# WHU-USI3DV/LaneMapping

Hardware: AMD Instinct MI355X
Metric: BEV tiles/sec end-to-end (LAS points -> polylines) (higher is better)
Workload: dtype f32; 1 GPU; on-GPU LAS->BEV raster (4,194,304 points/tile resident in HBM) + configs/Proj_polyline_fpn_vit_vertex_2.py, batch=16 per GPU, seeded random weights; lines_per_tile=45, streams=2, hip_graphs=True, points=resident, stream_check=not run (--full runs it), gather_check=n/a (1 rank), raster_check=not run (--full runs it), dist_ranks=1, rccl_ranks=1

## Files before the change

lanemapping_amd/csrc/conv_mfma.hip:

```cpp
#include "common.h"

#include <cstdlib>

typedef float f32x16 __attribute__((ext_vector_type(16)));
typedef float f32x4 __attribute__((ext_vector_type(4)));

namespace {

constexpr int BK = 32;
constexpr int LDS_LD = BK;

__device__ __attribute__((aligned(16))) float g_zero_chunk[4] = {0.f, 0.f, 0.f, 0.f};

struct ConvParams {
    const float* x; const float* wp; const float* scale; const float* shift; const float* res; float* y;
    int ldx, ldr, ldy, res_rows;
    int B, H, W, Cin, Cout, CoutP, Ho, Wo;
    int KH, KW, stride, pad_h, pad_w, dil, act;
    long M;
    const float* zero;
    int taps_real;
    const int* nbr;
    double* gn_part;
    int gn_chunks;
// ... 246 lines not shown
                }
            }
        }
        if (p.gn_part) {
#pragma unroll
            for (int o = LPR; o < 64; o <<= 1)
#pragma unroll
                for (int e = 0; e < 4; ++e) {
                    gs[e] += __shfl_xor(gs[e], o);
                    gq[e] += __shfl_xor(gq[e], o);
                }
            if (lane < LPR) {
                const long hw = (long)p.Ho * p.Wo;
                const long mt = m0 + wm0;
                const long b = mt / hw;
                const long chunk = (mt - b * hw) / WM;
                double* o = p.gn_part + ((b * p.gn_chunks + chunk) * p.Cout + n) * 2;
                for (int e = 0; e < 4 && n + e < p.Cout; ++e) {
                    o[2 * e] = (double)gs[e];
                    o[2 * e + 1] = (double)gq[e];
                }
            }
        }
    }
}

template <int BM, int BN, int WM, int WN, bool GATHER = false, int TPS = 1>
int launch(const ConvParams& p, hipStream_t stream) {
    const size_t kloop = (size_t)2 * (BM + BN) * LDS_LD, stage = (size_t)((BM / WM) * (BN / WN)) * WM * (WN + 4);
    const size_t lds = (kloop > stage ? kloop : stage) * sizeof(float);
    if (int e = lm_ensure_dynamic_lds((const void*)conv_mfma_kernel<BM, BN, WM, WN, GATHER, TPS>, lds)) return e;
    const long m_tiles = (p.M + BM - 1) / BM;
    const long blocks = m_tiles * ((p.Cout + BN - 1) / BN);
    LM_REQUIRE(blocks > 0 && blocks < (1L << 31), "conv_mfma: bad grid %ld", blocks);
    hipLaunchKernelGGL((conv_mfma_kernel<BM, BN, WM, WN, GATHER, TPS>), dim3((unsigned)blocks), dim3((BM / WM) * (BN / WN) * 64), lds, stream, p);
    LM_LAUNCH_CHECK();
    return LM_OK;
}

constexpr int LAT_SLD = 36;
template <int KS, bool RESUP, bool ROWTILE>
__global__ __launch_bounds__(512) void lateral_mfma_kernel(ConvParams p) {
    constexpr int K = KS * 8, SLABS = K / 32, XBUF = 32 * K;
    constexpr int NX = XBUF / 4 / 512;
    static_assert(NX >= 1 && XBUF % (4 * 512) == 0, "whole load passes");
    extern __shared__ __attribute__((aligned(16))) float smem[];
    typedef __attribute__((address_space(1))) const void gptr_t;
    typedef __attribute__((address_space(3))) void lptr_t;
    const int tid = threadIdx.x, lane = tid & 63;
    const int wave = __builtin_amdgcn_readfirstlane(tid >> 6);
    const int j = lane & 31, half = lane >> 5;
    float* const patch = smem + 2 * XBUF + wave * (32 * LAT_SLD);
    f32x4 wf[KS];
    {
        const float* wrow = p.wp + (long)(wave * 32 + j) * p.Cin + 4 * half;
#pragma unroll
        for (int k = 0; k < KS; ++k) wf[k] = *reinterpret_cast<const f32x4*>(wrow + 8 * k);
    }
    const int erow = lane >> 3, n = wave * 32 + (lane & 7) * 4;
    const f32x4 sh = p.shift ? *reinterpret_cast<const f32x4*>(p.shift + n) : f32x4{0.f, 0.f, 0.f, 0.f};
    unsigned yoff[4], roff[4];
#pragma unroll
    for (int q = 0; q < 4; ++q) {
        yoff[q] = (unsigned)((erow + 8 * q) * p.ldy + n) * 4u;
        roff[q] = (unsigned)((erow + 8 * q) * p.ldr + n) * 4u;
    }
    const int ntiles = (int)(p.M >> 5);
    const int xcd = blockIdx.x & 7, wi = blockIdx.x >> 3, nwg = gridDim.x >> 3;
    const int per = (ntiles + 7) >> 3, t_end = min(ntiles, (xcd + 1) * per);
    int tile = xcd * per + wi;
    if (tile >= t_end) return;
    int xoff[NX];
#pragma unroll
    for (int i = 0; i < NX; ++i) {
        const int c = i * 512 + tid, slab = c >> 8, row = (c & 255) >> 3, slot = c & 7;
        xoff[i] = row * p.ldx + slab * 32 + ((slot ^ ((row >> 1) & 7)) << 2);
    }
    auto load_x = [&](int t, int buf) {
        const float* xt = p.x + (long)t * 32 * p.ldx;
#pragma unroll
        for (int i = 0; i < NX; ++i)
            __builtin_amdgcn_global_load_lds((gptr_t*)(xt + xoff[i]), (lptr_t*)(smem + buf * XBUF + (i * 8 + wave) * 256), 16, 0, 0);
    };
    load_x(tile, 0);
    __builtin_amdgcn_s_waitcnt(0x0F70);
    const int fswz = (j >> 1) & 7;
#pragma unroll
    for (int k = 0; k < KS; ++k) asm volatile("" : "+v"(wf[k]));
    for (int it = 0; tile < t_end; tile += nwg, ++it) {
        const int buf = it & 1;
        asm volatile("s_waitcnt vmcnt(4)" ::: "memory");
        __builtin_amdgcn_s_barrier();
        asm volatile("" ::: "memory");
        load_x(min(tile + nwg, t_end - 1), buf ^ 1);
        f32x4 r00[4], r01[4], r10[4], r11[4];
        float wy0[4], wy1[4], wx0[4], wx1[4];
        if (RESUP && ROWTILE) {
            const unsigned mt = (unsigned)__builtin_amdgcn_readfirstlane(tile) * 32u;
            const unsigned t = lm_fastdiv(mt, p.div_wo);
            const int ox0 = (int)(mt - t * p.div_wo.d);
            const int bi = (int)lm_fastdiv(t, p.div_ho);
            const int oy = (int)(t - (unsigned)bi * p.div_ho.d);
            int y0v, y1v;
            float wyav, wybv;
            lm_bilin_axis_scaled(oy, p.res_hi, p.res_sy, y0v, y1v, wyav, wybv);
            const int y0 = __builtin_amdgcn_readfirstlane(y0v), y1 = __builtin_amdgcn_readfirstlane(y1v);
            const float wya = __builtin_bit_cast(float, __builtin_amdgcn_readfirstlane(__builtin_bit_cast(int, wyav)));
            const float wyb = __builtin_bit_cast(float, __builtin_amdgcn_readfirstlane(__builtin_bit_cast(int, wybv)));
            const char* row0 = reinterpret_cast<const char*>(p.res + ((long)bi * p.res_hi + y0) * p.res_wi * p.ldr);
            const char* row1 = reinterpret_cast<const char*>(p.res + ((long)bi * p.res_hi + y1) * p.res_wi * p.ldr);
#pragma unroll
            for (int q = 0; q < 4; ++q) {
                int x0, x1;
                lm_bilin_axis_scaled(ox0 + erow + 8 * q, p.res_wi, p.res_sx, x0, x1, wx0[q], wx1[q]);
                wy0[q] = wya;
                wy1[q] = wyb;
                const unsigned o0 = (unsigned)(x0 * p.ldr + n) * 4u, o1 = (unsigned)(x1 * p.ldr + n) * 4u;
                r00[q] = *reinterpret_cast<const f32x4*>(row0 + o0);
                r01[q] = *reinterpret_cast<const f32x4*>(row0 + o1);
                r10[q] = *reinterpret_cast<const f32x4*>(row1 + o0);
                r11[q] = *reinterpret_cast<const f32x4*>(row1 + o1);
            }
        } else if (RESUP) {
#pragma unroll
            for (int q = 0; q < 4; ++q) {
                const unsigned m = (unsigned)(tile * 32 + erow + 8 * q);
                const unsigned t = lm_fastdiv(m, p.div_wo);
                const int ox = (int)(m - t * p.div_wo.d);
                const int bi = (int)lm_fastdiv(t, p.div_ho);
                const int oy = (int)(t - (unsigned)bi * p.div_ho.d);
                int y0, y1, x0, x1;
                lm_bilin_axis_scaled(oy, p.res_hi, p.res_sy, y0, y1, wy0[q], wy1[q]);
                lm_bilin_axis_scaled(ox, p.res_wi, p.res_sx, x0, x1, wx0[q], wx1[q]);
                const float* rb = p.res + (long)bi * p.res_hi * p.res_wi * p.ldr + n;
                r00[q] = *reinterpret_cast<const f32x4*>(rb + ((long)y0 * p.res_wi + x0) * p.ldr);
                r01[q] = *reinterpret_cast<const f32x4*>(rb + ((long)y0 * p.res_wi + x1) * p.ldr);
                r10[q] = *reinterpret_cast<const f32x4*>(rb + ((long)y1 * p.res_wi + x0) * p.ldr);
                r11[q] = *reinterpret_cast<const f32x4*>(rb + ((long)y1 * p.res_wi + x1) * p.ldr);
            }
        } else if (p.res_rows) {
#pragma unroll
            for (int q = 0; q < 4; ++q) {
                const unsigned m = (unsigned)(tile * 32 + erow + 8 * q);
                r00[q] = *reinterpret_cast<const f32x4*>(p.res + (long)(m - lm_fastdiv(m, p.div_rr) * p.div_rr.d) * p.ldr + n);
            }
        } else {
            const char* rt = reinterpret_cast<const char*>(p.res + (long)__builtin_amdgcn_readfirstlane(tile) * 32 * p.ldr);
#pragma unroll
            for (int q = 0; q < 4; ++q) r00[q] = *reinterpret_cast<const f32x4*>(rt + roff[q]);
        }
        __builtin_amdgcn_sched_barrier(0);
        f32x16 acc;
#pragma unroll
        for (int r = 0; r < 16; ++r) acc[r] = 0.f;
        const float* xb = smem + buf * XBUF + j * 32;
        f32x4 xf = *reinterpret_cast<const f32x4*>(xb + ((half ^ fswz) << 2));
#pragma unroll
        for (int k = 0; k < KS; ++k) {
            f32x4 xn = xf;
            acc = __builtin_amdgcn_mfma_f32_32x32x2f32(wf[k][0], xf[0], acc, 0, 0, 0);
            if (k + 1 < KS) {
                const int fo = (((((k + 1) & 3) << 1) + half) ^ fswz) << 2;
                __builtin_amdgcn_sched_barrier(0);
                xn = *reinterpret_cast<const f32x4*>(xb + ((k + 1) >> 2) * 1024 + fo);
                __builtin_amdgcn_sched_barrier(0);
            }
#pragma unroll
            for (int t = 1; t < 4; ++t) acc = __builtin_amdgcn_mfma_f32_32x32x2f32(wf[k][t], xf[t], acc, 0, 0, 0);
            xf = xn;
        }
        __builtin_amdgcn_sched_barrier(0);
#pragma unroll
        for (int g = 0; g < 4; ++g)
            *reinterpret_cast<f32x4*>(patch + j * LAT_SLD + 8 * g + 4 * half) = f32x4{acc[4 * g], acc[4 * g + 1], acc[4 * g + 2], acc[4 * g + 3]};
        char* const yt = reinterpret_cast<char*>(p.y + (long)__builtin_amdgcn_readfirstlane(tile) * 32 * p.ldy);
#pragma unroll
        for (int q = 0; q < 4; ++q) {
            f32x4 v = *reinterpret_cast<const f32x4*>(patch + (erow + 8 * q) * LAT_SLD + (lane & 7) * 4);
#pragma unroll
            for (int e = 0; e < 4; ++e) v[e] = v[e] + sh[e];
            if (RESUP) {
#pragma unroll
                for (int e = 0; e < 4; ++e) v[e] += lm_bilerp(r00[q][e], r01[q][e], r10[q][e], r11[q][e], wy0[q], wy1[q], wx0[q], wx1[q]);
            } else {
#pragma unroll
                for (int e = 0; e < 4; ++e) v[e] += r00[q][e];
            }
            *reinterpret_cast<f32x4*>(yt + yoff[q]) = v;
        }
    }
}

int lateral_try(const ConvParams& p, hipStream_t stream) {
    static const int on = [] { const char* e = getenv("LM_CONV_LATERAL"); return e ? atoi(e) : 1; }();
    if (!on || p.KH != 1 || p.KW != 1 || p.stride != 1 || p.pad_h != 0 || p.pad_w != 0 || p.Cout != 256 || p.CoutP != 256) return 0;
    if ((p.Cin != 64 && p.Cin != 128) || p.scale || p.act != LM_ACT_NONE || p.gn_part || !p.res) return 0;
    if ((p.ldx & 3) || (p.ldy & 3) || (p.ldr & 3) || p.ldr < p.Cout || p.M >= (1L << 31) - 64 || (p.M & 31)) return 0;
    if (p.res_hi > 0 && p.Cin != 64) return 0;
    if (p.res_hi == 0 && p.Cin != 128) return 0;
    static int cus = 0;
    if (!cus) {
        int dev = 0;
        hipDeviceProp_t prop;
        if (hipGetDevice(&dev) != hipSuccess || hipGetDeviceProperties(&prop, dev) != hipSuccess) return -LM_ERR_HIP;
        cus = prop.multiProcessorCount > 0 ? prop.multiProcessorCount : 256;
    }
    const int ntiles = (int)((p.M + 31) / 32);
    int grid = (cus + 7) / 8 * 8;
    if (grid > (ntiles + 7) / 8 * 8) grid = (ntiles + 7) / 8 * 8;
    const size_t lds = (size_t)(2 * 32 * p.Cin + 8 * 32 * LAT_SLD) * sizeof(float);
#define LM_LAT_LAUNCH(KS, UP, ROW)                                                                                      \
    {                                                                                                                   \
        if (lm_ensure_dynamic_lds((const void*)lateral_mfma_kernel<KS, UP, ROW>, lds)) return -LM_ERR_HIP;              \
        hipLaunchKernelGGL((lateral_mfma_kernel<KS, UP, ROW>), dim3(grid), dim3(512), lds, stream, p);                  \
    }
    if (p.res_hi > 0 && p.Wo % 32 == 0) LM_LAT_LAUNCH(8, true, true)
    else if (p.res_hi > 0) LM_LAT_LAUNCH(8, true, false)
    else LM_LAT_LAUNCH(16, false, false)
#undef LM_LAT_LAUNCH
    if (hipGetLastError() != hipSuccess) return -LM_ERR_HIP;
    return 1;
}

int zero_block(const float** out) {
    static const float* ptr = nullptr;
    if (!ptr) {
        void* sym = nullptr;
        LM_HIP(hipGetSymbolAddress(&sym, HIP_SYMBOL(g_zero_chunk)));
        ptr = (const float*)sym;
    }
    *out = ptr;
    return LM_OK;
}

}

static int conv_dispatch(void* stream, const float* x, int ldx, const float* wp, int CoutP, const float* scale, const float* shift,
                         const float* res, int ldr, int res_rows, float* y, int ldy, int B, int H, int W, int Cin, int Cout,
                         int KH, int KW, int stride, int pad_h, int pad_w, int dil, int act, double* gn_part, int res_hi = 0,
                         int res_wi = 0) {
    LM_REQUIRE(x && wp && y, "conv_mfma: null pointer");
    LM_REQUIRE(Cin > 0 && Cin % BK == 0, "conv_mfma: Cin=%d must be a multiple of %d", Cin, BK);
    LM_REQUIRE(CoutP >= Cout && CoutP % 128 == 0, "conv_mfma: CoutP=%d must be Cout=%d rounded up to 128", CoutP, Cout);
    LM_REQUIRE(ldx >= Cin && ldx % 4 == 0 && ldy >= Cout, "conv_mfma: bad leading dims ldx=%d ldy=%d", ldx, ldy);
    LM_REQUIRE(stride >= 1 && dil >= 1 && KH >= 1 && KW >= 1, "conv_mfma: bad geometry");
    ConvParams p;
    p.x = x; p.wp = wp; p.scale = scale; p.shift = shift; p.res = res; p.y = y;
    p.ldx = ldx; p.ldr = ldr; p.ldy = ldy; p.res_rows = res_rows;
    p.res_hi = res_hi; p.res_wi = res_wi;
    p.B = B; p.H = H; p.W = W; p.Cin = Cin; p.Cout = Cout; p.CoutP = CoutP;
    p.Ho = (H + 2 * pad_h - dil * (KH - 1) - 1) / stride + 1;
    p.Wo = (W + 2 * pad_w - dil * (KW - 1) - 1) / stride + 1;
    LM_REQUIRE(p.Ho > 0 && p.Wo > 0, "conv_mfma: empty output");
    p.KH = KH; p.KW = KW; p.stride = stride; p.pad_h = pad_h; p.pad_w = pad_w; p.dil = dil; p.act = act;
    p.M = (long)B * p.Ho * p.Wo;
    LM_REQUIRE(((long)B * H * W + (long)(KH * dil + pad_h + 1) * W) * ldx < (1L << 31) && (long)KH * KW * CoutP * Cin < (1L << 31),
               "conv_mfma: tensor too large for 32-bit element offsets (B*H*W*ld = %ld)", (long)B * H * W * ldx);
    p.gn_part = gn_part;
    p.gn_chunks = 0;
    p.nbr = nullptr;
    p.taps_real = 0;
    LM_REQUIRE(p.M < (1L << 31) && res_rows >= 0, "conv_mfma: %ld output pixels do not fit 32-bit indices", p.M);
    p.div_wo = lm_fastdiv_make((unsigned)p.Wo);
    p.div_ho = lm_fastdiv_make((unsigned)p.Ho);
    p.div_rr = lm_fastdiv_make((unsigned)(res_rows > 0 ? res_rows : 1));
    p.res_sy = (res_hi > 0 && p.Ho > 1) ? (float)(res_hi - 1) / (float)(p.Ho - 1) : 0.f;
    p.res_sx = (res_wi > 0 && p.Wo > 1) ? (float)(res_wi - 1) / (float)(p.Wo - 1) : 0.f;
    if (int e = zero_block(&p.zero)) return e;
    hipStream_t s = (hipStream_t)stream;
    {
        const int r = lateral_try(p, s);
        if (r < 0) {
            lm_set_error("conv_mfma: lateral kernel launch failed");
            return -r;
        }
        if (r > 0) return LM_OK;
    }
    if (gn_part) {
        LM_REQUIRE(Cout > 64 && Cout % 4 == 0 && ((long)p.Ho * p.Wo) % 128 == 0 && res == nullptr && act == LM_ACT_NONE,
                   "conv_mfma(gn stats): needs Cout > 64, Ho*Wo %% 128 == 0, no residual / activation");
        p.gn_chunks = (int)((long)p.Ho * p.Wo / 64);
        return launch<128, 128, 64, 64>(p, s);
    }
    if (Cout <= 64) return launch<128, 64, 32, 64>(p, s);
    {
        static const long tiny_k = [] { const char* e = getenv("LM_CONV_TINYK"); return e ? atol(e) : 256L; }();
        if ((long)KH * KW * Cin <= tiny_k) return launch<128, 128, 32, 64>(p, s);
    }
    const long big_blocks = ((p.M + 127) / 128) * ((Cout + 127) / 128);
    static const long small_m = [] { const char* e = getenv("LM_CONV_SMALLM"); return e ? atol(e) : 700L; }();
    if (big_blocks < small_m) return launch<64, 64, 32, 32>(p, s);
    return launch<128, 128, 64, 64>(p, s);
}

LM_API int lm_conv2d_nhwc_mfma_f32(void* stream, const float* x, int ldx, const float* wp, int CoutP,
                                   const float* scale, const float* shift,
                                   const float* res, int ldr, int res_rows, float* y, int ldy,
                                   int B, int H, int W, int Cin, int Cout, int KH, int KW,
                                   int stride, int pad_h, int pad_w, int dil, int act) {
    return conv_dispatch(stream, x, ldx, wp, CoutP, scale, shift, res, ldr, res_rows, y, ldy, B, H, W, Cin, Cout, KH, KW, stride,
                         pad_h, pad_w, dil, act, nullptr);
}

LM_API int lm_conv2d_nhwc_mfma_f32_gnstats(void* stream, const float* x, int ldx, const float* wp, int CoutP, const float* shift,
                                           float* y, int ldy, double* gn_partial, int B, int H, int W, int Cin, int Cout,
                                           int KH, int KW, int stride, int pad_h, int pad_w, int dil) {
    LM_REQUIRE(gn_partial, "conv_mfma(gn stats): null partial buffer");
    return conv_dispatch(stream, x, ldx, wp, CoutP, nullptr, shift, nullptr, 0, 0, y, ldy, B, H, W, Cin, Cout, KH, KW, stride,
                         pad_h, pad_w, dil, LM_ACT_NONE, gn_partial);
}

LM_API int lm_conv2d_nhwc_mfma_resup_f32(void* stream, const float* x, int ldx, const float* wp, int CoutP, const float* scale,
                                         const float* shift, const float* res_coarse, int ldr, int Hr, int Wr, float* y, int ldy,
                                         int B, int H, int W, int Cin, int Cout, int KH, int KW, int stride, int pad_h, int pad_w,
                                         int dil, int act) {
    LM_REQUIRE(res_coarse && Hr > 0 && Wr > 0, "conv_mfma(resup): missing coarse residual");
    LM_REQUIRE(Cout % 4 == 0 && ldy % 4 == 0 && ldr % 4 == 0 && ldr >= Cout, "conv_mfma(resup): Cout=%d, ldy=%d, ldr=%d must be multiples of 4", Cout, ldy, ldr);
    const long Ho = (H + 2 * pad_h - dil * (KH - 1) - 1) / stride + 1, Wo = (W + 2 * pad_w - dil * (KW - 1) - 1) / stride + 1;
    LM_REQUIRE((long)B * Ho * Wo < (1L << 31), "conv_mfma(resup): too many output pixels for 32-bit indices");
    return conv_dispatch(stream, x, ldx, wp, CoutP, scale, shift, res_coarse, ldr, 0, y, ldy, B, H, W, Cin, Cout, KH, KW, stride,
                         pad_h, pad_w, dil, act, nullptr, Hr, Wr);
}

LM_API int lm_conv_gather_mfma_f32(void* stream, const float* x, int ldx, const int* nbr, int taps, const float* wp, int CoutP,
                                   const float* scale, const float* shift, const float* res, int ldr, float* y, int ldy,
                                   long M, int Cin, int Cout, int act) {
    LM_REQUIRE(x && nbr && wp && y, "conv_gather: null pointer");
    LM_REQUIRE(M > 0 && taps >= 1, "conv_gather: empty problem (M=%ld taps=%d)", M, taps);
    LM_REQUIRE(Cin == 16 || (Cin > 0 && Cin % BK == 0), "conv_gather: Cin=%d must be 16 or a multiple of %d (zero-pad the feature rows)",
               Cin, BK);
    LM_REQUIRE(CoutP >= Cout && CoutP % 128 == 0, "conv_gather: CoutP=%d must be Cout=%d rounded up to 128", CoutP, Cout);
    LM_REQUIRE(ldx >= Cin && ldx % 4 == 0 && ldy >= Cout, "conv_gather: bad leading dims ldx=%d ldy=%d", ldx, ldy);
    const bool pairs = Cin == 16;
    const int slabs = pairs ? (taps + 1) / 2 : taps;
    ConvParams p;
    p.x = x; p.wp = wp; p.scale = scale; p.shift = shift; p.res = res; p.y = y;
    p.ldx = ldx; p.ldr = ldr; p.ldy = ldy; p.res_rows = 0;
    p.res_hi = 0; p.res_wi = 0;
    p.B = 1; p.H = 1; p.W = 1; p.Cin = pairs ? BK : Cin; p.Cout = Cout; p.CoutP = CoutP; p.Ho = 1; p.Wo = 1;
    p.KH = 1; p.KW = slabs; p.stride = 1; p.pad_h = 0; p.pad_w = 0; p.dil = 1; p.act = act;
    p.M = M;
    LM_REQUIRE(M < (1L << 31) && (long)slabs * CoutP * p.Cin < (1L << 31), "conv_gather: problem too large (M=%ld)", M);
    p.gn_part = nullptr;
    p.gn_chunks = 0;
    p.div_wo = p.div_ho = p.div_rr = lm_fastdiv_make(1);
    p.res_sy = p.res_sx = 0.f;
    p.nbr = nbr;
    p.taps_real = taps;
    if (int e = zero_block(&p.zero)) return e;
    hipStream_t s = (hipStream_t)stream;
    if (pairs) {
        if (Cout <= 32) return launch<128, 32, 32, 32, true, 2>(p, s);
        return launch<128, 64, 32, 64, true, 2>(p, s);
    }
    if (Cout <= 32) return launch<128, 32, 32, 32, true>(p, s);
    if (Cout <= 64) return launch<128, 64, 32, 64, true>(p, s);
    return launch<128, 128, 64, 64, true>(p, s);
}
```

lanemapping_amd/csrc/conv_wino44.hip:

```cpp
#include "common.h"

#include <cstdlib>

typedef float f32x16 __attribute__((ext_vector_type(16)));
typedef float f32x4 __attribute__((ext_vector_type(4)));
typedef float f32x2 __attribute__((ext_vector_type(2)));
typedef _Float16 f16x4 __attribute__((ext_vector_type(4)));
typedef unsigned u32x2 __attribute__((ext_vector_type(2)));

namespace {

__device__ __forceinline__ u32x2 w44_split2(f32x2 t) {
#pragma clang fp contract(off)
    typedef __fp16 f16x2r __attribute__((ext_vector_type(2)));
    const f16x2r h = __builtin_amdgcn_cvt_pkrtz(t[0], t[1]);
    const float h0 = (float)h[0], h1 = (float)h[1];
    const f16x2r l = __builtin_amdgcn_cvt_pkrtz(t[0] - h0, t[1] - h1);
    return u32x2{__builtin_bit_cast(unsigned, h), __builtin_bit_cast(unsigned, l)};
}

constexpr int QBM = 32, QBN = 64, QSEG = 4;
constexpr int QNCELL = 144;
constexpr int QLPW = 14;
constexpr int QGRP = 256 + 8;
constexpr int QRAWF = QLPW * 4 * QGRP;
constexpr int QVF = 36 * 256;
constexpr int QBD = 5, QRING = 6;
static_assert(6 * (QNCELL / 16) * QGRP <= QRAWF && QNCELL % 16 == 0, "patch loads cover the unit");

constexpr unsigned QPADOFF = 0x80000000u;
typedef __amdgpu_buffer_rsrc_t w44_rsrc_t;

struct W44Geom {
    int B, H, W, dil, Ty, Tx;
    int Timg, Tpad;
    long T;
    LmFastDiv dTx, dTy, ddil, dTpad;
};

W44Geom geom44(int B, int H, int W, int dil) {
    W44Geom g;
    g.B = B; g.H = H; g.W = W; g.dil = dil;
    g.Ty = ((H + dil - 1) / dil + 3) / 4;
    g.Tx = ((W + dil - 1) / dil + 3) / 4;
    g.Timg = dil * dil * g.Ty * g.Tx;
    g.Tpad = (g.Timg + QBM - 1) / QBM * QBM;
    g.T = (long)B * g.Tpad;
    g.dTx = lm_fastdiv_make((unsigned)g.Tx); g.dTy = lm_fastdiv_make((unsigned)g.Ty);
    g.ddil = lm_fastdiv_make((unsigned)dil); g.dTpad = lm_fastdiv_make((unsigned)g.Tpad);
    return g;
}

__device__ __forceinline__ void tile44_decode(const W44Geom& g, int t, int& pa, int& pb, int& ty, int& tx) {
    tx = t % g.Tx;
    t /= g.Tx;
    ty = t % g.Ty;
    const int ph = t / g.Ty;
    pa = ph / g.dil;
    pb = ph - pa * g.dil;
}

__device__ __forceinline__ void w44_bt(const float (&d)[6], float (&t)[6]) {
#pragma clang fp contract(off)
    t[0] = __builtin_fmaf(4.f, d[0], __builtin_fmaf(-5.f, d[2], d[4]));
    t[5] = __builtin_fmaf(4.f, d[1], __builtin_fmaf(-5.f, d[3], d[5]));
    const float p = __builtin_fmaf(-4.f, d[2], d[4]), q = __builtin_fmaf(-4.f, d[1], d[3]);
    t[1] = p + q;
    t[2] = p - q;
    const float r = d[4] - d[2], s = d[3] - d[1];
    t[3] = __builtin_fmaf(2.f, s, r);
    t[4] = __builtin_fmaf(-2.f, s, r);
}

__device__ __forceinline__ float w44_fma(float k, float a, float c) { return __builtin_fmaf(k, a, c); }
__device__ __forceinline__ f32x4 w44_fma(float k, f32x4 a, f32x4 c) { return __builtin_elementwise_fma(f32x4{k, k, k, k}, a, c); }
template <typename T>
__device__ __forceinline__ void w44_at(const T (&m)[6], T (&y)[4]) {
#pragma clang fp contract(off)
    const T s1 = m[1] + m[2], d1 = m[1] - m[2], s3 = m[3] + m[4], d3 = m[3] - m[4];
    y[0] = (m[0] + s1) + s3;
    y[1] = w44_fma(2.f, d3, d1);
    y[2] = w44_fma(4.f, s3, s1);
    y[3] = w44_fma(8.f, d3, d1) + m[5];
}

// ... 307 lines not shown
    return 2 * QBD + c;
}
static_assert(q_dma0(17) + q_ndma(17) == QLPW, "the second phase issues every patch load of a unit");

template <bool SPLIT>
__device__ __forceinline__ f32x4 q_aread(const float* v, const float* v1) {
    if constexpr (SPLIT) {
        return f32x4{v[0], v[32], v[128], v[160]};
    } else {
        const f32x2 lo = *reinterpret_cast<const f32x2*>(v), hi = *reinterpret_cast<const f32x2*>(v1);
        return f32x4{lo[0], lo[1], hi[0], hi[1]};
    }
}

__device__ __forceinline__ float* w44_lds_hide(float* p) {
    typedef __attribute__((address_space(3))) float lds_float;
    unsigned a = (unsigned)(unsigned long)(lds_float*)p;
    asm volatile("" : "+v"(a));
    return (float*)(lds_float*)(unsigned long)a;
}

constexpr bool w44_deferred(int S) { return S == 4 || S == 8 || S == 13; }
template <int S>
__device__ __forceinline__ void w44_step_rest(f32x16& acc0, f32x16& acc1, const f32x4 (&b)[2], const f32x4& a_cur) {
    constexpr bool VACC = S % 9 == 8;
    q_mfma<VACC>(acc1, a_cur[0], b[1][0]);
#pragma unroll
    for (int t = 1; t < 4; ++t) {
        q_mfma<VACC>(acc0, a_cur[t], b[0][t]);
        q_mfma<VACC>(acc1, a_cur[t], b[1][t]);
    }
}

template <int S, bool SPLIT>
__device__ __forceinline__ void w44_step(f32x16& acc0, f32x16& acc1, f32x4 (&bq)[QRING][2], unsigned bvoff, const float* bpre,
                                         const float* anext, const float* anext1, const f32x4& a_cur, f32x4& a_nxt, const w44_rsrc_t grsrc, const unsigned (&gvoff)[QLPW], int gsoff,
                                         float* rawld, int wave, W44Xf& xf, const float* const (&col)[6], float* vA, float* vB,
                                         float* vC, bool lower, const W44K& kk) {
    typedef __attribute__((address_space(3))) void lptr_t;
    constexpr int K = S % 9;
    q_bload2(bq[(S + QBD) % QRING], bvoff, bpre);
#pragma unroll
    for (int i = 0; i < q_ndma(S); ++i) {
        constexpr int L0 = q_dma0(S);
        __builtin_amdgcn_raw_ptr_buffer_load_lds(grsrc, (lptr_t*)(rawld + ((L0 + i) * 4 + wave) * QGRP), 16, gvoff[L0 + i], gsoff, 0, 0);
    }
    f32x4 (&b)[2] = bq[S % QRING];
    q_bwait<q_nwait(S)>(b);
    constexpr bool VACC = K == 8;
    const f32x2 a_hi = {a_cur[0], a_cur[1]}, a_lo = {a_cur[2], a_cur[3]};
    if constexpr (SPLIT) q_mfma16<VACC>(acc0, a_hi, f32x2{b[0][0], b[0][1]});
    else q_mfma<VACC>(acc0, a_cur[0], b[0][0]);
    if constexpr (!SPLIT) __builtin_amdgcn_sched_barrier(0);
    if constexpr (K != 4 && K != 8) a_nxt = q_aread<SPLIT>(anext, anext1);
    w44_xf_lds<K, SPLIT>(xf, col, vA, vB, vC);
    if constexpr (!SPLIT) __builtin_amdgcn_sched_barrier(0);
    w44_xf_valu<K>(xf, lower, kk);
    if constexpr (!SPLIT) __builtin_amdgcn_sched_barrier(0);
    if constexpr (SPLIT) {
        q_mfma16<VACC>(acc1, a_hi, f32x2{b[1][0], b[1][1]});
        q_mfma16<VACC>(acc0, a_hi, f32x2{b[0][2], b[0][3]});
        q_mfma16<VACC>(acc1, a_hi, f32x2{b[1][2], b[1][3]});
        q_mfma16<VACC>(acc0, a_lo, f32x2{b[0][0], b[0][1]});
        q_mfma16<VACC>(acc1, a_lo, f32x2{b[1][0], b[1][1]});
        if constexpr (!VACC) {
#pragma unroll
            for (int i = 0; i < 6; ++i) {
                __builtin_amdgcn_sched_group_barrier(0x008, 1, 0);
                __builtin_amdgcn_sched_group_barrier(0x002, 6, 0);
                __builtin_amdgcn_sched_group_barrier(0x300, 3, 0);
            }
        }
    } else if constexpr (!w44_deferred(S)) {
        w44_step_rest<S>(acc0, acc1, b, a_cur);
    }
    __builtin_amdgcn_sched_barrier(0);
}

__device__ __forceinline__ float w44_vmax(float a, float b) {
    float r;
    asm("v_max_f32 %0, %1, %2" : "=v"(r) : "v"(a), "v"(b));
    return r;
}
template <bool FULL>
__device__ __forceinline__ void w44_tail_vec(const f32x4 (&z)[4][6], const f32x4 (&rpre)[16], float* yp, int rowstep, int colstep, const f32x4 sc,
                                             const f32x4 sh, float relu_lo, bool has_res, bool gn, f32x4& gsum, f32x4& gsq, int eny, int enx) {
#pragma unroll
    for (int yy = 0; yy < 4; ++yy) {
        f32x4 o[4];
        w44_at(z[yy], o);
#pragma unroll
        for (int xx = 0; xx < 4; ++xx) {
#pragma clang fp contract(off)
            if (!FULL && !(yy < eny && xx < enx)) continue;
            f32x4 v = o[xx] * sc + sh;
            if (gn) {
#pragma unroll
                for (int e = 0; e < 4; ++e) {
                    gsum[e] += v[e];
                    gsq[e] = __builtin_fmaf(v[e], v[e], gsq[e]);
                }
            }
            if (has_res) v += rpre[yy * 4 + xx];
#pragma unroll
            for (int e = 0; e < 4; ++e) v[e] = w44_vmax(v[e], relu_lo);
            *reinterpret_cast<f32x4*>(yp + yy * rowstep + xx * colstep) = v;
        }
    }
}

template <bool SPLIT>
__global__ __launch_bounds__(256) void wino44_kernel(W44Params p) {
    extern __shared__ __attribute__((aligned(16))) float smem[];
    float* const raw0 = smem;
    float* const Vbuf = smem + 2 * QRAWF;
    typedef __attribute__((address_space(3))) void lptr_t;
    const int tid = threadIdx.x, lane = tid & 63;
    const int wave = __builtin_amdgcn_readfirstlane(tid >> 6);
    const int n_tiles = (p.Cout + QBN - 1) / QBN;
    unsigned mblk, ntile;
    if (p.n_inner) {
        const unsigned bid = blockIdx.x, per = gridDim.x / 8;
        const unsigned lin = bid < per * 8 ? (bid % 8) * per + bid / 8 : bid;
        mblk = lm_fastdiv(lin, p.dnt);
        ntile = lin - mblk * (unsigned)n_tiles;
    } else {
        const unsigned bid = blockIdx.x, mb = gridDim.x / (unsigned)n_tiles, mbx = mb / 8, full = mbx * 8 * (unsigned)n_tiles;
        if (bid < full) {
            const unsigned xcd = bid % 8, idx = bid / 8;
            ntile = idx / mbx;
            mblk = xcd * mbx + idx % mbx;
        } else {
            const unsigned r = bid - full;
            mblk = 8 * mbx + r / (unsigned)n_tiles;
            ntile = r % (unsigned)n_tiles;
        }
    }
    const long m0 = (long)mblk * QBM;
    const int n0 = (int)ntile * QBN;
    const W44Geom& g = p.g;
    const int bi = (int)lm_fastdiv((unsigned)m0, g.dTpad);
    const int t0 = (int)(m0 - (long)bi * g.Tpad);
    int ts[QSEG + 1], sn[QSEG], iy0[QSEG], ix0[QSEG], oy0[QSEG], ox0[QSEG];
    {
        int at = 0, t = t0;
        const int rest = (int)lm_fastdiv((unsigned)t0, g.dTx), ph = (int)lm_fastdiv((unsigned)rest, g.dTy);
        int tx = t0 - rest * g.Tx, ty = rest - ph * g.Ty;
        int pa = (int)lm_fastdiv((unsigned)ph, g.ddil), pb = ph - pa * g.dil;
#pragma unroll
        for (int s_ = 0; s_ < QSEG; ++s_) {
            ts[s_] = at;
            const bool real = t < g.Timg && at < QBM;
            const int n = at < QBM ? min(QBM - at, g.Tx - tx) : 0;
            sn[s_] = real ? n : 0;
            iy0[s_] = (4 * ty - 1) * g.dil + pa;
            ix0[s_] = (4 * tx - 1) * g.dil + pb;
            oy0[s_] = 4 * ty * g.dil + pa;
            ox0[s_] = 4 * tx * g.dil + pb;
            at += n;
            t += n;
            tx += n;
            if (tx >= g.Tx) {
                tx = 0;
                if (++ty >= g.Ty) {
                    ty = 0;
                    if (++pb >= g.dil) {
// ... 91 lines not shown
    for (int k = 0; k < 9; ++k)
#pragma unroll
        for (int b = 0; b < 2; ++b)
#pragma unroll
            for (int r = 0; r < 16; ++r) acc[k][b][r] = 0.f;
    f32x4 bq[QRING][2];
    W44Xf xf;
#define LM_QXI(K) (6 * ((K) / 3) + (K) % 3)
#pragma unroll
    for (int k = 0; k < QBD; ++k) q_bload2(bq[k], bvoff, bbase + (long)LM_QXI(k) * xstride);
    {
        const int gsoff1 = nun > 1 ? 64 : 0;
#pragma unroll
        for (int s_ = 0; s_ < QLPW; ++s_)
            __builtin_amdgcn_raw_ptr_buffer_load_lds(grsrc, (lptr_t*)(raw0 + QRAWF + (s_ * 4 + wave) * QGRP), 16, gvoff[s_], gsoff1, 0, 0);
    }
    q_bwait<QLPW>(bq[0]);
    __builtin_amdgcn_s_barrier();
    {
        const float* const col0[6] = LM_QCOLS(0, 0);
        w44_xf_all<SPLIT>(xf, col0, vA, vB, vC, lower, kk);
    }
    asm volatile("s_waitcnt lgkmcnt(0)" ::: "memory");
    __builtin_amdgcn_s_barrier();

#define LM_QBPRE(S5) ((S5) < 18 ? bu + (long)((S5) / 9) * ustride + (long)LM_QXI((S5) % 9) * xstride : bu_next + (long)LM_QXI((S5) - 18) * xstride)
#define LM_QANEXT(S) (LM_QXI(((S) % 9) + 1 < 9 ? ((S) % 9) + 1 : 0) * 256)
#define LM_QSTEP(S, AC, AN) \
    w44_step<S, SPLIT>(acc[(S) % 9][0], acc[(S) % 9][1], bq, bvoff, LM_QBPRE((S) + QBD), Vq + LM_QANEXT(S), Vq1 + LM_QANEXT(S), \
                AC, AN, grsrc, gvoff, gsoff, rawc_w, wave, xf, (S) < 9 ? colc : coln, vA, vB, vC, lower, kk)
#define LM_QMID(AN)                                          \
    asm volatile("s_waitcnt lgkmcnt(0)" ::: "memory");       \
    __builtin_amdgcn_s_barrier();                            \
    AN = q_aread<SPLIT>(Vq + LM_QXI(5) * 256, Vq1 + LM_QXI(5) * 256); \
    __builtin_amdgcn_sched_barrier(0);
#define LM_QREST(S, AC)                                                                               \
    if constexpr (!SPLIT) {                                                                           \
        w44_step_rest<S>(acc[(S) % 9][0], acc[(S) % 9][1], bq[(S) % QRING], AC);                      \
        __builtin_amdgcn_sched_barrier(0);                                                            \
    }
    auto unit = [&](auto par_, const int u) __attribute__((always_inline)) {
        constexpr int PAR = decltype(par_)::value;
        const float* const colc[6] = LM_QCOLS(PAR, 8);
        const float* const coln[6] = LM_QCOLS(PAR ^ 1, 0);
        float* const rawc_w = raw0 + PAR * QRAWF;
        const int gsoff = u + 2 < nun ? (u + 2) * 64 : 0;
        const float* const bu = bbase + (long)(2 * u) * ustride;
        const float* const bu_next = bbase + (long)(u + 1 < nun ? 2 * (u + 1) : 0) * ustride;
        f32x4 a0, a1;
        a0 = q_aread<SPLIT>(Vq, Vq1);
        LM_QSTEP(0, a0, a1); LM_QSTEP(1, a1, a0); LM_QSTEP(2, a0, a1); LM_QSTEP(3, a1, a0); LM_QSTEP(4, a0, a1);
        LM_QMID(a1)
        LM_QREST(4, a0)
        LM_QSTEP(5, a1, a0); LM_QSTEP(6, a0, a1); LM_QSTEP(7, a1, a0); LM_QSTEP(8, a0, a1);
        asm volatile("s_waitcnt lgkmcnt(0)" ::: "memory");
        q_bwait<2 * 9>(bq[0]);
        __builtin_amdgcn_s_barrier();
        a1 = q_aread<SPLIT>(Vq, Vq1);
        __builtin_amdgcn_sched_barrier(0);
        LM_QREST(8, a0)
        LM_QSTEP(9, a1, a0);  LM_QSTEP(10, a0, a1); LM_QSTEP(11, a1, a0); LM_QSTEP(12, a0, a1); LM_QSTEP(13, a1, a0);
        LM_QMID(a0)
        LM_QREST(13, a1)
        LM_QSTEP(14, a0, a1); LM_QSTEP(15, a1, a0); LM_QSTEP(16, a0, a1); LM_QSTEP(17, a1, a0);
        asm volatile("s_waitcnt lgkmcnt(0)" ::: "memory");
        __builtin_amdgcn_s_barrier();
    };
    for (int u = 0; u + 1 < nun; u += 2) {
        unit(W44Int<0>{}, u);
        unit(W44Int<1>{}, u + 1);
    }
    if (nun & 1) unit(W44Int<0>{}, nun - 1);
#undef LM_QCOLS
#undef LM_QCOL
#undef LM_QREST
#undef LM_QMID
#undef LM_QSTEP
#undef LM_QANEXT
#undef LM_QBPRE
#undef LM_QXI
    static_assert(18 % QRING == 0 && QBD < QRING, "eighteen steps per unit walk the ring a whole number of times");
#pragma unroll
    for (int k = 0; k < QRING; ++k) q_bwait<0>(bq[k]);

    const int elane = (int)__builtin_amdgcn_mbcnt_hi(~0u, __builtin_amdgcn_mbcnt_lo(~0u, 0u)), etid = wave * 64 + elane;
    const int etile = etid >> 3, ecq = etid & 7;
    int epix0;
    int eny = 0, enx = 0;
    {
        int nn = sn[0], oy = oy0[0], oxb = ox0[0], tb = 0;
#pragma unroll
        for (int k = 1; k < QSEG; ++k)
            if (etile >= ts[k]) {
                nn = sn[k]; oy = oy0[k]; oxb = ox0[k]; tb = ts[k];
            }
        const int ox = oxb + 4 * (etile - tb) * g.dil;
        epix0 = img_pix0 + oy * g.W + ox;
        if (nn > 0 && oy < g.H && ox < g.W) {
            eny = min(4, (int)lm_fastdiv((unsigned)(g.H - oy + g.dil - 1), g.ddil));
            enx = min(4, (int)lm_fastdiv((unsigned)(g.W - ox + g.dil - 1), g.ddil));
        }
    }
    float* const mw = smem + xi00 * 1024 + (4 * (elane >> 5)) * 32 + (elane & 31);
    const float* const mr = smem + etile * 32 + ecq * 4;
    f32x4 gsum[2] = {{0.f, 0.f, 0.f, 0.f}, {0.f, 0.f, 0.f, 0.f}}, gsq[2] = {{0.f, 0.f, 0.f, 0.f}, {0.f, 0.f, 0.f, 0.f}};
    const bool full = eny == 4 && enx == 4;
    const int ebase = eny > 0 ? epix0 : img_pix0;
    const int ey1 = max(eny - 1, 0), ex1 = max(enx - 1, 0);
    const float relu_lo = p.act == LM_ACT_RELU ? 0.f : -__builtin_inff();
    const bool has_res = p.res != nullptr, gn = p.gn_part != nullptr;
#pragma unroll
    for (int blk = 0; blk < 2; ++blk) {
        const int n = n0 + blk * 32 + ecq * 4;
        const bool vec = (n + 3 < p.Cout) && ((p.ldy & 3) == 0) && (!p.res || (p.ldr & 3) == 0);
        f32x4 sc = {1.f, 1.f, 1.f, 1.f}, sh = {0.f, 0.f, 0.f, 0.f};
        if (vec) {
            if (p.scale) sc = *reinterpret_cast<const f32x4*>(p.scale + n);
            if (p.shift) sh = *reinterpret_cast<const f32x4*>(p.shift + n);
            if constexpr (SPLIT) sc = sc * p.post;
        } else {
#pragma unroll
            for (int e = 0; e < 4; ++e)
                if (n + e < p.Cout) {
                    if (p.scale) sc[e] = p.scale[n + e];
                    if (p.shift) sh[e] = p.shift[n + e];
                    if constexpr (SPLIT) sc[e] = sc[e] * p.post;
                }
        }
        f32x4 rpre[16];
        const bool load_res = vec && has_res;
        const float* const rp = p.res + (long)ebase * p.ldr + n;
        const int rs = g.W * g.dil * p.ldr, cs = g.dil * p.ldr;
        asm volatile("s_waitcnt lgkmcnt(0)" ::: "memory");
        __builtin_amdgcn_s_barrier();
#pragma unroll
        for (int k = 0; k < 9; ++k) {
#pragma unroll
            for (int r = 0; r < 16; ++r) mw[(6 * (k / 3) + k % 3) * 1024 + ((r & 3) + 8 * (r >> 2)) * 32] = acc[k][blk][r];
            if (k < 8 && load_res) {
#pragma unroll
                for (int q = 2 * k; q < 2 * k + 2; ++q)
                    rpre[q] = *reinterpret_cast<const f32x4*>(rp + min(q >> 2, ey1) * rs + min(q & 3, ex1) * cs);
            }
            __builtin_amdgcn_sched_barrier(0);
        }
        asm volatile("s_waitcnt lgkmcnt(0)" ::: "memory");
        __builtin_amdgcn_s_barrier();
        if (n < p.Cout && eny > 0) {
            f32x4 z[4][6];
#pragma unroll
            for (int j = 0; j < 6; ++j) {
                f32x4 col[6], y4[4];
#pragma unroll
                for (int i = 0; i < 6; ++i) col[i] = *reinterpret_cast<const f32x4*>(mr + (6 * i + j) * 1024);
                w44_at(col, y4);
#pragma unroll
                for (int yy = 0; yy < 4; ++yy) z[yy][j] = y4[yy];
            }
            float* const yp = p.y + (long)ebase * p.ldy + n;
            const int rowstep = g.W * g.dil * p.ldy, colstep = g.dil * p.ldy;
            if (vec) {
                if (full) w44_tail_vec<true>(z, rpre, yp, rowstep, colstep, sc, sh, relu_lo, has_res, gn, gsum[blk], gsq[blk], eny, enx);
                else w44_tail_vec<false>(z, rpre, yp, rowstep, colstep, sc, sh, relu_lo, has_res, gn, gsum[blk], gsq[blk], eny, enx);
            } else {
#pragma unroll
                for (int yy = 0; yy < 4; ++yy) {
                    f32x4 o[4];
                    w44_at(z[yy], o);
#pragma unroll
                    for (int xx = 0; xx < 4; ++xx) {
#pragma clang fp contract(off)
                        const f32x4 v = o[xx] * sc + sh;
#pragma unroll
                        for (int e = 0; e < 4; ++e) {
                            if (!(yy < eny && xx < enx && n + e < p.Cout)) continue;
                            if (gn) {
                                gsum[blk][e] += v[e];
                                gsq[blk][e] = __builtin_fmaf(v[e], v[e], gsq[blk][e]);
                            }
                            float u = v[e];
                            if (has_res) u += p.res[((long)ebase + (yy * g.W + xx) * g.dil) * p.ldr + n + e];
                            yp[yy * rowstep + xx * colstep + e] = fmaxf(u, relu_lo);
                        }
                    }
                }
            }
        }
    }
    if (p.gn_part) {
#pragma unroll
        for (int blk = 0; blk < 2; ++blk)
#pragma unroll
            for (int o = 8; o < 64; o <<= 1)
#pragma unroll
                for (int e = 0; e < 4; ++e) {
                    gsum[blk][e] += __shfl_xor(gsum[blk][e], o);
                    gsq[blk][e] += __shfl_xor(gsq[blk][e], o);
                }
        __syncthreads();
        if (elane < 8) {
#pragma unroll
            for (int blk = 0; blk < 2; ++blk) {
                *reinterpret_cast<f32x4*>(smem + (((wave * 2 + blk) * 8 + elane) * 2) * 4) = gsum[blk];
                *reinterpret_cast<f32x4*>(smem + (((wave * 2 + blk) * 8 + elane) * 2 + 1) * 4) = gsq[blk];
            }
        }
        __syncthreads();
        if (etid < 16) {
#pragma clang fp contract(off)
            const int blk = etid >> 3, cq = etid & 7;
            const int n = n0 + blk * 32 + cq * 4;
            f32x4 s = {0.f, 0.f, 0.f, 0.f}, q = {0.f, 0.f, 0.f, 0.f};
#pragma unroll
            for (int w = 0; w < 4; ++w) {
                const f32x4 a = *reinterpret_cast<const f32x4*>(smem + (((w * 2 + blk) * 8 + cq) * 2) * 4);
                const f32x4 b = *reinterpret_cast<const f32x4*>(smem + (((w * 2 + blk) * 8 + cq) * 2 + 1) * 4);
#pragma unroll
                for (int e = 0; e < 4; ++e) {
                    s[e] += a[e];
                    q[e] += b[e];
                }
            }
            const long chunk = t0 / 32;
            double* o = p.gn_part + (((long)bi * (g.Tpad / 32) + chunk) * p.Cout + n) * 2;
            for (int e = 0; e < 4 && n + e < p.Cout; ++e) {
                o[2 * e] = (double)s[e];
                o[2 * e + 1] = (double)q[e];
            }
        }
    }
}

bool w44_ok(const W44Geom& g) { return (QBM - 2) / g.Tx + 2 <= QSEG; }

bool w44_image_ok(int H, int W, int Cin, int ldx) { return ((long)H * W - 1) * ldx * 4 + (long)Cin * 4 < (1L << 31); }

}

LM_API int lm_winograd44_supported_ld(int H, int W, int Cin, int dil, int ldx) {
    if (dil < 1 || H < 1 || W < 1 || Cin < 16 || Cin % 16 != 0 || Cin > 1024 || ldx < Cin) return 0;
    return w44_ok(geom44(1, H, W, dil)) && w44_image_ok(H, W, Cin, ldx) ? 1 : 0;
}

LM_API int lm_winograd44_supported(int H, int W, int Cin, int dil) { return lm_winograd44_supported_ld(H, W, Cin, dil, Cin); }

LM_API int lm_winograd44_gn_chunks(int H, int W, int dil) { return dil < 1 ? 0 : geom44(1, H, W, dil).Tpad / 32; }

LM_API long lm_winograd44_tiles(int B, int H, int W, int dil) { return dil < 1 ? 0 : geom44(B, H, W, dil).T; }

LM_API long lm_winograd44_twin_workspace_bytes(int B, int H, int W, int Cin, int CoutP, int dil) {
    if (dil < 1) return 0;
    return 36 * geom44(B, H, W, dil).T * (long)(Cin + CoutP) * (long)sizeof(float);
}

static int w44_launch(void* stream, const float* x, int ldx, const float* wu_frag, int CoutP, const float* scale,
                      const float* shift, const float* res, int ldr, float* y, int ldy, int B, int H, int W,
                      int Cin, int Cout, int dil, int act, double* gn_partial, float split_post) {
    LM_REQUIRE(x && wu_frag && y, "conv_wino44: null pointer");
    LM_REQUIRE(lm_winograd44_supported(H, W, Cin, dil) && B > 0, "conv_wino44: unsupported shape (H=%d W=%d Cin=%d dil=%d)", H, W, Cin, dil);
    LM_REQUIRE(w44_image_ok(H, W, Cin, ldx), "conv_wino44: an image of the input spans 2^31 bytes or more (H=%d W=%d ldx=%d): use the direct kernel", H, W, ldx);
    LM_REQUIRE(CoutP >= Cout && CoutP % QBN == 0, "conv_wino44: CoutP=%d must be Cout=%d rounded up to %d", CoutP, Cout, QBN);
    LM_REQUIRE(ldx >= Cin && ldx % 4 == 0 && ldy >= Cout, "conv_wino44: bad leading dimension");
    LM_REQUIRE(act == LM_ACT_NONE || act == LM_ACT_RELU, "conv_wino44: activation %d not supported", act);
    LM_REQUIRE(!gn_partial || (res == nullptr && act == LM_ACT_NONE && Cout % 4 == 0), "conv_wino44(gn stats): no residual / activation");
    W44Params p;
    p.g = geom44(B, H, W, dil);
    LM_REQUIRE((long)B * H * W * ldx < (1L << 40) && (long)B * H * W < (1L << 31) && p.g.T < (1L << 31), "conv_wino44: tensor too large");
    p.x = x; p.U = wu_frag; p.scale = scale; p.shift = shift; p.res = res; p.y = y;
    p.ldx = ldx; p.ldr = ldr; p.ldy = ldy; p.C = Cin; p.Cout = Cout; p.NT = CoutP / 32; p.act = act;
    p.gn_part = gn_partial;
    static const int order = getenv("LANEMAP_W44_ORDER") ? atoi(getenv("LANEMAP_W44_ORDER")) : 1;
    p.n_inner = order;
    p.dnt = lm_fastdiv_make((unsigned)((Cout + QBN - 1) / QBN));
    const size_t lds = (size_t)(2 * QRAWF + QVF) * sizeof(float);
    static_assert(36 * 32 * 32 <= 2 * QRAWF + QVF, "the product buffer of the epilogue fits");
    const long blocks = (p.g.T / QBM) * ((Cout + QBN - 1) / QBN);
    LM_REQUIRE(blocks > 0 && blocks < (1L << 31) && p.g.T % QBM == 0, "conv_wino44: bad grid %ld", blocks);
    p.post = split_post != 0.f ? split_post : 1.f;
    if (split_post != 0.f) {
        if (int e = lm_ensure_dynamic_lds((const void*)wino44_kernel<true>, lds)) return e;
        hipLaunchKernelGGL(wino44_kernel<true>, dim3((unsigned)blocks), dim3(256), lds, (hipStream_t)stream, p);
    } else {
        if (int e = lm_ensure_dynamic_lds((const void*)wino44_kernel<false>, lds)) return e;
        hipLaunchKernelGGL(wino44_kernel<false>, dim3((unsigned)blocks), dim3(256), lds, (hipStream_t)stream, p);
    }
    LM_LAUNCH_CHECK();
    return LM_OK;
}

LM_API int lm_conv3x3_winograd44_f32(void* stream, const float* x, int ldx, const float* wu_frag, int CoutP, const float* scale,
                                     const float* shift, const float* res, int ldr, float* y, int ldy, int B, int H, int W,
                                     int Cin, int Cout, int dil, int act, double* gn_partial) {
    return w44_launch(stream, x, ldx, wu_frag, CoutP, scale, shift, res, ldr, y, ldy, B, H, W, Cin, Cout, dil, act, gn_partial, 0.f);
}

LM_API int lm_conv3x3_winograd44_split_f32(void* stream, const float* x, int ldx, const float* wu_split, int CoutP, const float* scale,
                                           const float* shift, const float* res, int ldr, float* y, int ldy, int B, int H, int W,
                                           int Cin, int Cout, int dil, int act, double* gn_partial, float post) {
    LM_REQUIRE(post > 0.f, "conv_wino44(split): post scale must be positive");
// ... 55 lines not shown
```

Measured before the change: 395.4 tiles/s.

## Tabulate lateral bilinear x-offsets in LDS, retune conv tiles, asm-driven Winograd accumulator exchange

In the row-tiled lateral upsample kernel, the per-column bilinear x indices and weights are now precomputed once per block into an LDS table and prefetched for the next tile, so the inner loop no longer recomputes them. The launcher adds LDS for that table and limits the row-tile path to Wo<=4096. The conv tile chooser gets an LM_CONV_TILE env override and picks a 128x64 tile for tiny-K convs whose Cout remainder is small. The Winograd 4x4 kernel writes accumulator planes with inline ds_write_b32 asm using immediate offsets straight from AGPRs, and inserts s_nops after the barrier waits. It also simplifies the GroupNorm partial-sum LDS indexing.

```diff
diff --git a/lanemapping_amd/csrc/conv_mfma.hip b/lanemapping_amd/csrc/conv_mfma.hip
--- a/lanemapping_amd/csrc/conv_mfma.hip
+++ b/lanemapping_amd/csrc/conv_mfma.hip
@@ -352,6 +352,27 @@
         for (int i = 0; i < NX; ++i)
             __builtin_amdgcn_global_load_lds((gptr_t*)(xt + xoff[i]), (lptr_t*)(smem + buf * XBUF + (i * 8 + wave) * 256), 16, 0, 0);
     };
+    typedef unsigned u32x4 __attribute__((ext_vector_type(4)));
+    const u32x4* xt_lane = nullptr;
+    u32x4 tx[4];
+    auto tab_read = [&](int t, u32x4 (&d)[4]) {
+        const unsigned mt = (unsigned)__builtin_amdgcn_readfirstlane(t) * 32u;
+        const unsigned ox0 = mt - lm_fastdiv(mt, p.div_wo) * p.div_wo.d;
+#pragma unroll
+        for (int q = 0; q < 4; ++q) d[q] = xt_lane[ox0 + 8 * q];
+    };
+    if (RESUP && ROWTILE) {
+        u32x4* const xtab = reinterpret_cast<u32x4*>(smem + 2 * XBUF + 8 * (32 * LAT_SLD));
+        for (int ox = tid; ox < p.Wo; ox += 512) {
+            int x0, x1;
+            float w0, w1;
+            lm_bilin_axis_scaled(ox, p.res_wi, p.res_sx, x0, x1, w0, w1);
+            xtab[ox] = u32x4{(unsigned)(x0 * p.ldr) * 4u, (unsigned)(x1 * p.ldr) * 4u, __builtin_bit_cast(unsigned, w0), __builtin_bit_cast(unsigned, w1)};
+        }
+        __syncthreads();
+        xt_lane = xtab + erow;
+        tab_read(tile, tx);
+    }
     load_x(tile, 0);
     __builtin_amdgcn_s_waitcnt(0x0F70);
     const int fswz = (j >> 1) & 7;
@@ -368,7 +389,6 @@
         if (RESUP && ROWTILE) {
             const unsigned mt = (unsigned)__builtin_amdgcn_readfirstlane(tile) * 32u;
             const unsigned t = lm_fastdiv(mt, p.div_wo);
-            const int ox0 = (int)(mt - t * p.div_wo.d);
             const int bi = (int)lm_fastdiv(t, p.div_ho);
             const int oy = (int)(t - (unsigned)bi * p.div_ho.d);
             int y0v, y1v;
@@ -381,16 +401,18 @@
             const char* row1 = reinterpret_cast<const char*>(p.res + ((long)bi * p.res_hi + y1) * p.res_wi * p.ldr);
 #pragma unroll
             for (int q = 0; q < 4; ++q) {
-                int x0, x1;
-                lm_bilin_axis_scaled(ox0 + erow + 8 * q, p.res_wi, p.res_sx, x0, x1, wx0[q], wx1[q]);
+                const unsigned w0b = tx[q][2], w1b = tx[q][3];
+                wx0[q] = __builtin_bit_cast(float, w0b);
+                wx1[q] = __builtin_bit_cast(float, w1b);
                 wy0[q] = wya;
                 wy1[q] = wyb;
-                const unsigned o0 = (unsigned)(x0 * p.ldr + n) * 4u, o1 = (unsigned)(x1 * p.ldr + n) * 4u;
+                const unsigned o0 = tx[q][0] + (unsigned)n * 4u, o1 = tx[q][1] + (unsigned)n * 4u;
                 r00[q] = *reinterpret_cast<const f32x4*>(row0 + o0);
                 r01[q] = *reinterpret_cast<const f32x4*>(row0 + o1);
                 r10[q] = *reinterpret_cast<const f32x4*>(row1 + o0);
                 r11[q] = *reinterpret_cast<const f32x4*>(row1 + o1);
             }
+            tab_read(min(tile + nwg, t_end - 1), tx);
         } else if (RESUP) {
 #pragma unroll
             for (int q = 0; q < 4; ++q) {
@@ -478,13 +500,14 @@
     const int ntiles = (int)((p.M + 31) / 32);
     int grid = (cus + 7) / 8 * 8;
     if (grid > (ntiles + 7) / 8 * 8) grid = (ntiles + 7) / 8 * 8;
-    const size_t lds = (size_t)(2 * 32 * p.Cin + 8 * 32 * LAT_SLD) * sizeof(float);
+    const bool rowtile = p.res_hi > 0 && p.Wo % 32 == 0 && p.Wo <= 4096;
+    const size_t lds = (size_t)(2 * 32 * p.Cin + 8 * 32 * LAT_SLD + (rowtile ? 4 * p.Wo : 0)) * sizeof(float);
 #define LM_LAT_LAUNCH(KS, UP, ROW)                                                                                      \
     {                                                                                                                   \
         if (lm_ensure_dynamic_lds((const void*)lateral_mfma_kernel<KS, UP, ROW>, lds)) return -LM_ERR_HIP;              \
         hipLaunchKernelGGL((lateral_mfma_kernel<KS, UP, ROW>), dim3(grid), dim3(512), lds, stream, p);                  \
     }
-    if (p.res_hi > 0 && p.Wo % 32 == 0) LM_LAT_LAUNCH(8, true, true)
+    if (rowtile) LM_LAT_LAUNCH(8, true, true)
     else if (p.res_hi > 0) LM_LAT_LAUNCH(8, true, false)
     else LM_LAT_LAUNCH(16, false, false)
 #undef LM_LAT_LAUNCH
@@ -553,9 +576,17 @@
         return launch<128, 128, 64, 64>(p, s);
     }
     if (Cout <= 64) return launch<128, 64, 32, 64>(p, s);
+    static const int force_tile = [] { const char* e = getenv("LM_CONV_TILE"); return e ? atoi(e) : 0; }();
+    switch (force_tile) {
+        case 1: return launch<64, 64, 32, 32>(p, s);
+        case 2: return launch<128, 64, 32, 64>(p, s);
+        case 3: return launch<128, 128, 64, 64>(p, s);
+        case 4: return launch<128, 128, 32, 64>(p, s);
+        default: break;
+    }
     {
         static const long tiny_k = [] { const char* e = getenv("LM_CONV_TINYK"); return e ? atol(e) : 256L; }();
-        if ((long)KH * KW * Cin <= tiny_k) return launch<128, 128, 32, 64>(p, s);
+        if ((long)KH * KW * Cin <= tiny_k) return (Cout - 1) % 128 < 64 ? launch<128, 64, 32, 64>(p, s) : launch<128, 128, 32, 64>(p, s);
     }
     const long big_blocks = ((p.M + 127) / 128) * ((Cout + 127) / 128);
     static const long small_m = [] { const char* e = getenv("LM_CONV_SMALLM"); return e ? atol(e) : 700L; }();
diff --git a/lanemapping_amd/csrc/conv_wino44.hip b/lanemapping_amd/csrc/conv_wino44.hip
--- a/lanemapping_amd/csrc/conv_wino44.hip
+++ b/lanemapping_amd/csrc/conv_wino44.hip
@@ -1,6 +1,7 @@
 #include "common.h"
 
 #include <cstdlib>
+#include <utility>
 
 typedef float f32x16 __attribute__((ext_vector_type(16)));
 typedef float f32x4 __attribute__((ext_vector_type(4)));
@@ -474,6 +475,16 @@
     asm("v_max_f32 %0, %1, %2" : "=v"(r) : "v"(a), "v"(b));
     return r;
 }
+template <int OFF>
+__device__ __forceinline__ void w44_xchg_acc(unsigned addr, float v) {
+    static_assert(OFF >= 0 && OFF < (1 << 16), "ds offset field");
+    asm volatile("ds_write_b32 %0, %1 offset:%2" : : "v"(addr), "a"(v), "n"(OFF) : "memory");
+}
+template <int K, int... R>
+__device__ __forceinline__ void w44_xchg_plane(unsigned addr, const f32x16& a, std::integer_sequence<int, R...>) {
+    (w44_xchg_acc<((6 * (K / 3) + K % 3) * 1024 + ((R & 3) + 8 * (R >> 2)) * 32) * 4>(addr, a[R]), ...);
+}
+
 template <bool FULL>
 __device__ __forceinline__ void w44_tail_vec(const f32x4 (&z)[4][6], const f32x4 (&rpre)[16], float* yp, int rowstep, int colstep, const f32x4 sc,
                                              const f32x4 sh, float relu_lo, bool has_res, bool gn, f32x4& gsum, f32x4& gsq, int eny, int enx) {
@@ -731,6 +742,7 @@
     static_assert(18 % QRING == 0 && QBD < QRING, "eighteen steps per unit walk the ring a whole number of times");
 #pragma unroll
     for (int k = 0; k < QRING; ++k) q_bwait<0>(bq[k]);
+    asm volatile("s_nop 15\n\ts_nop 3");
 
     const int elane = (int)__builtin_amdgcn_mbcnt_hi(~0u, __builtin_amdgcn_mbcnt_lo(~0u, 0u)), etid = wave * 64 + elane;
     const int etile = etid >> 3, ecq = etid & 7;
@@ -751,6 +763,8 @@
         }
     }
     float* const mw = smem + xi00 * 1024 + (4 * (elane >> 5)) * 32 + (elane & 31);
+    typedef __attribute__((address_space(3))) float w44_lds_float;
+    const unsigned mwa = (unsigned)(unsigned long)(w44_lds_float*)mw;
     const float* const mr = smem + etile * 32 + ecq * 4;
     f32x4 gsum[2] = {{0.f, 0.f, 0.f, 0.f}, {0.f, 0.f, 0.f, 0.f}}, gsq[2] = {{0.f, 0.f, 0.f, 0.f}, {0.f, 0.f, 0.f, 0.f}};
     const bool full = eny == 4 && enx == 4;
@@ -782,17 +796,23 @@
         const int rs = g.W * g.dil * p.ldr, cs = g.dil * p.ldr;
         asm volatile("s_waitcnt lgkmcnt(0)" ::: "memory");
         __builtin_amdgcn_s_barrier();
-#pragma unroll
-        for (int k = 0; k < 9; ++k) {
-#pragma unroll
-            for (int r = 0; r < 16; ++r) mw[(6 * (k / 3) + k % 3) * 1024 + ((r & 3) + 8 * (r >> 2)) * 32] = acc[k][blk][r];
+        auto xchg = [&](auto kc) {
+            constexpr int k = decltype(kc)::value;
+            if constexpr (k < 8) {
+                w44_xchg_plane<k>(mwa, acc[k][blk], std::make_integer_sequence<int, 16>{});
+            } else {
+#pragma unroll
+                for (int r = 0; r < 16; ++r) mw[(6 * (k / 3) + k % 3) * 1024 + ((r & 3) + 8 * (r >> 2)) * 32] = acc[k][blk][r];
+            }
             if (k < 8 && load_res) {
 #pragma unroll
                 for (int q = 2 * k; q < 2 * k + 2; ++q)
                     rpre[q] = *reinterpret_cast<const f32x4*>(rp + min(q >> 2, ey1) * rs + min(q & 3, ex1) * cs);
             }
             __builtin_amdgcn_sched_barrier(0);
-        }
+        };
+        xchg(W44Int<0>{}); xchg(W44Int<1>{}); xchg(W44Int<2>{}); xchg(W44Int<3>{}); xchg(W44Int<4>{});
+        xchg(W44Int<5>{}); xchg(W44Int<6>{}); xchg(W44Int<7>{}); xchg(W44Int<8>{});
         asm volatile("s_waitcnt lgkmcnt(0)" ::: "memory");
         __builtin_amdgcn_s_barrier();
         if (n < p.Cout && eny > 0) {
@@ -862,8 +882,8 @@
             f32x4 s = {0.f, 0.f, 0.f, 0.f}, q = {0.f, 0.f, 0.f, 0.f};
 #pragma unroll
             for (int w = 0; w < 4; ++w) {
-                const f32x4 a = *reinterpret_cast<const f32x4*>(smem + (((w * 2 + blk) * 8 + cq) * 2) * 4);
-                const f32x4 b = *reinterpret_cast<const f32x4*>(smem + (((w * 2 + blk) * 8 + cq) * 2 + 1) * 4);
+                const f32x4 a = *reinterpret_cast<const f32x4*>(smem + ((w * 16 + etid) * 2) * 4);
+                const f32x4 b = *reinterpret_cast<const f32x4*>(smem + ((w * 16 + etid) * 2 + 1) * 4);
 #pragma unroll
                 for (int e = 0; e < 4; ++e) {
                     s[e] += a[e];
```

Measured after the change: 396.5 tiles/s (median of 4 runs). About the same (+0.3%).
